# caomw/ClusteringSegmentation-1

Hardware: AMD Instinct MI355X
Metric: Mpixels/sec DivQuant K=256 on 3840x2160 RGB (higher is better)
Workload: dtype u8 RGB (packed u32 frames, planar u8 working buffers), u32/u64 integer sums, f64 updates; 1 GPU; C4 per-GPU share: 8 x 3840x2160 frames per rank per step, K=256, quant_recurse max_iters=10 (cluster + dedup + map), one batched call; engine_lanes=4, gpu_max_hw_queues=8, gpu_max_hw_queues_set_by_bench=True, width=3840, height=2160, k=256, max_iters=10, parallelism=frames-per-rank x1

## Files before the change

### clusteringsegmentation-1_amd/csrc/dq_abi.cpp

```cpp
#include <hip/hip_runtime.h>

#include <algorithm>
#include <cmath>
#include <cstdio>
#include <cstdlib>
#include <cstring>
#include <atomic>
#include <condition_variable>
#include <functional>
#include <mutex>
#include <thread>
#include <unordered_map>
#include <vector>

#include "../../include/DivQuantHeader.h"
#include "../../include/dq_hip.h"
#include "../../include/quant_util.h"
#include "dq_engine.h"
#include "dq_adjacency.h"
#include "dq_merge.h"
#include "dq_regions.h"
#include "dq_weighted.h"

#include <rccl/rccl.h>
// ... 323 lines not shown
  return 0;
}

static int quant_batch(int device, std::vector<dq::FrameJob>& jobs, int max_iters, void* stream) {
  const int nframes = (int)jobs.size();
  const int lanes = std::min(nframes, dq::batch_lanes());
  Engine& e0 = engine_for(device);
  if (lanes <= 1) {
    std::lock_guard<std::mutex> g(e0.mutex());
    e0.run(jobs.data(), nframes, max_iters, true, dev_stream(e0, stream));
  } else {
    DQ_HIP(hipSetDevice(device));
    hipEvent_t ready = events().get();
    DQ_HIP(hipEventRecord(ready, (hipStream_t)stream));
    for (int l = 1; l < lanes; ++l) {
      Engine& e = engine_for(device, l);
      e.set_fixed_point(e0.fixed_point());
      e.set_plan(e0.plan());
      e.set_timing(e0.timing());
    }
    const std::function<void(int)> work = [&](int l) {
      const int f0 = nframes * l / lanes, f1 = nframes * (l + 1) / lanes;
      Engine& e = engine_for(device, l);
      DQ_HIP(hipSetDevice(device));
      std::lock_guard<std::mutex> g(e.mutex());
      DQ_HIP(hipStreamWaitEvent(e.stream(), ready, 0));
      e.run(jobs.data() + f0, f1 - f0, max_iters, true, e.stream());
    };
    lane_workers().run(lanes, work);
    events().put(ready);
    Engine& el = engine_for(device, lanes - 1);
    std::lock_guard<std::mutex> g(e0.mutex());
    uint64_t swept = 0, full = 0, fixes = 0;
    int rounds = 0;
    for (int l = 0; l < lanes; ++l) {
      Engine& e = engine_for(device, l);
      swept += e.last_points_swept;
      full += e.last_points_full;
      fixes += e.last_cursor_fixes;
      rounds = std::max(rounds, e.last_rounds);
      if (l > 0) e0.absorb_stats(e);
    }
    e0.last_means = el.last_means;
    e0.last_sizes = el.last_sizes;
    e0.last_trace = el.last_trace;
    e0.last_rounds = rounds;
    e0.last_points_swept = swept;
    e0.last_points_full = full;
    e0.last_cursor_fixes = fixes;
  }
  int empty = 0;
  for (int i = 0; i < nframes; ++i) empty += jobs[i].num_empty;
  return empty;
}

int dq_hip_quant_batch_dev(int device, int nframes, const uint32_t* const* d_in,
                           const uint32_t* n, uint32_t* const* d_out, uint32_t k,
                           uint32_t* ct, uint32_t* k_out, int max_iters, void* stream) {
  if (nframes <= 0 || !d_in || !n || !d_out || !ct || !k_out || k == 0 || max_iters < 1)
    return -1;
  for (int i = 0; i < nframes; ++i)
    if (!d_in[i] || !d_out[i] || n[i] == 0) return -1;
  std::vector<dq::FrameJob> jobs(nframes);
  for (int i = 0; i < nframes; ++i) {
    jobs[i].d_in = d_in[i];
    jobs[i].n = n[i];
    jobs[i].d_out = d_out[i];
    jobs[i].k = (int)k;
    jobs[i].ct = ct + (size_t)i * k;
  }
  const int empty = quant_batch(device, jobs, max_iters, stream);
  for (int i = 0; i < nframes; ++i) k_out[i] = (uint32_t)jobs[i].k_out;
  return empty;
}

int dq_hip_quant_bgr24_batch_dev(int device, int nframes, const uint8_t* const* d_bgr, uint32_t width,
                                 uint32_t height, uint32_t stride, uint32_t* const* d_out, uint32_t k,
                                 uint32_t* ct, uint32_t* k_out, int uniq, int max_iters, void* stream) {
  if (nframes <= 0 || !d_bgr || !d_out || !ct || !k_out || k == 0 || max_iters < 1 ||
// ... 993 lines not shown
```

### clusteringsegmentation-1_amd/csrc/dq_engine.cpp

```cpp
#include "dq_engine.h"
#include "dq_rules.h"
#include "dq_weighted.h"

#include <rccl/rccl.h>

#include <algorithm>
#include <cfloat>
#include <cmath>
#include <cstdio>
#include <cstdlib>
#include <cstring>
#include <map>
#include <atomic>
#include <chrono>
#include <deque>
#include <functional>
#include <string>
#include <unordered_map>

namespace dq {

void die(const char* what, const char* file, int line, const char* detail) {
  std::fprintf(stderr, "divquant-hip: fatal: %s (%s:%d): %s\n", what, file, line,
               detail ? detail : "");
// ... 395 lines not shown
const uint8_t* Engine::buf_ptr(int buf, const FrameState& f, int shard) const {
  if (buf == BUF_IN) return reinterpret_cast<const uint8_t*>(f.in[shard]);
  return reinterpret_cast<const uint8_t*>(buf == BUF_P0 ? d_p0_ : d_p1_) + f.base[shard];
}

uint64_t Engine::round_tile_len(uint64_t total) const {
  uint64_t tl = (total + tiles_target_ - 1) / tiles_target_;
  tl = ((tl + kSweep - 1) / kSweep) * kSweep;
  return std::max<uint64_t>(kSweep, std::min<uint64_t>(tl, tile_max_));
}

int Engine::src_fmt(const std::vector<int>& ids) const {
  int f = -1;
  for (int id : ids) {
    const Node& n = nodes_[id];
    const int g = n.buf != BUF_IN ? FMT_PLANAR : (frames_[n.frame].job->bgr ? FMT_BGR : FMT_PACKED);
    if (f >= 0 && g != f) return FMT_ANY;
    f = g;
  }
  return f < 0 ? FMT_ANY : f;
}

Engine::RoundBlock Engine::round_block(size_t nr, size_t tiles, size_t ptiles, size_t extra, int max_iters) {
  auto al = [](size_t x) { return (x + 63) & ~(size_t)63; };
  RoundBlock b;
  b.o_tiles = al(nr * sizeof(DevNode));
  b.o_pt = b.o_tiles + al(tiles * sizeof(Tile));
  b.o_extra = b.o_pt + al(ptiles * sizeof(PartTile));
  b.o_ctr = b.o_extra + al(extra);
  b.o_wp = b.o_ctr + al((size_t)(max_iters + 1) * sizeof(LaunchCtr));
  b.o_rd = b.o_wp + al(tiles * kTileWaves * sizeof(uint32_t));
  b.o_sum = b.o_rd + al((size_t)max_iters * nr * sizeof(uint32_t));
  b.o_sd = b.o_sum + al(nr * sizeof(RecSummary));
  b.bytes = b.o_sd + al(nr * sizeof(uint32_t));
  return b;
}

void Engine::round_args(Round& R, char* dblk, const RoundBlock& b, int mode) {
  RoundArgs& ra = R.ra;
  ra.tiles = R.dt;
  ra.nodes = R.dn;
  ra.parts = d_parts_;
  ra.parts2 = d_parts2_;
  ra.wparts = reinterpret_cast<uint32_t*>(dblk + b.o_wp);
  ra.ptiles = reinterpret_cast<const PartTile*>(dblk + b.o_pt);
  ra.sparts = d_sparts_;
  ra.hres = d_res_ + (size_t)R.par * cap_res_;
  ra.ctr = reinterpret_cast<LaunchCtr*>(dblk + b.o_ctr);
  ra.hstat = d_stat_ + (size_t)R.par * cap_stat_;
  ra.seq = R.seq;
  ra.fixed_point = fixed_point_ ? 1 : 0;
  ra.nn = R.nr;
  ra.tot = d_tot_;
  ra.nshard = nshard_;
  ra.debug = debug_;
  ra.rdone = reinterpret_cast<uint32_t*>(dblk + b.o_rd);
  ra.rsum = reinterpret_cast<RecSummary*>(dblk + b.o_sum);
  ra.dres = d_dres_ + (size_t)R.par * cap_res_;
  ra.plane = cap_px_;
  ra.tot_mode = mode;
}

int Engine::enqueue_host_round(const std::vector<int>& active_in, bool root_round, int max_iters,
                               hipStream_t stream) {
  debug_host_delay();
  const double tb0 = trace_ ? host_us() : 0.0;
  const int S = nshard_;
  const int mode = tot_mode();
  rounds_.emplace_back();
  const int ri = (int)rounds_.size() - 1;
  Round& R = rounds_[ri];
  R.root = root_round;
  std::vector<int>& order = R.order;
  std::vector<int>& parents = R.parents;
  slot_of_.assign(nodes_.size(), -1);
  parent_pos_.assign(nodes_.size(), -1);
  for (int id : active_in)
    if (root_round || nodes_[nodes_[id].parent].partitioned) order.push_back(id);
  const int n_own = (int)order.size();
  for (int id : active_in) {
    if (root_round || nodes_[nodes_[id].parent].partitioned) continue;
    order.push_back(id);
    const int p = nodes_[id].parent;
    if (parent_pos_[p] < 0) {
      parent_pos_[p] = (int)parents.size();
      parents.push_back(p);
    }
  }
  const int nl = (int)order.size();
// ... 21 lines not shown
  double own_bytes = 0.0, part_bytes = 0.0;
  for (int a = 0; a < nl; ++a)
    for (int sh = 0; sh < S; ++sh) {
      total += seg(order[a], sh).len;
      if (a < n_own) {
        own_total += seg(order[a], sh).len;
        own_bytes += point_bytes(order[a]) * seg(order[a], sh).len;
      }
    }
  for (int p : parents)
    for (int sh = 0; sh < S; ++sh) {
      parent_total += seg(p, sh).len;
      part_bytes += (point_bytes(p) + 3.0) * seg(p, sh).len;
    }
  const uint64_t tl = round_tile_len(total);
  size_t ntiles = 0, nt_own = 0;
  for (int a = 0; a < nl; ++a) {
    for (int sh = 0; sh < S; ++sh) ntiles += ntiles_of(seg(order[a], sh).len, (uint32_t)tl, (uint32_t)node_tiles_);
    if (a == n_own - 1) nt_own = ntiles;
  }
  size_t nptiles = 0;
  for (int p : parents)
    for (int sh = 0; sh < S; ++sh) nptiles += seg(p, sh).ntiles;
  DQ_CHECK(ntiles <= cap_parts_ && 2 * nptiles <= cap_sparts_, "round larger than the run's tile capacity");
  R.total = total;
  R.own_total = own_total;
  R.parent_total = parent_total;
  R.tl = tl;
  R.ntiles = R.tiles_cap = ntiles;
  R.nptiles = R.ptiles_cap = nptiles;
  R.nt_own = nt_own;

  const RoundBlock blk = round_block((size_t)nr, ntiles, nptiles, nmat * sizeof(PartTile), max_iters);
  const size_t bytes = blk.bytes;
  R.bytes = bytes;
  if (mode == TOT_ALLREDUCE) ensure_totals(nl, stream);
  if (stage_pending_) {
    DQ_HIP(hipEventSynchronize(stage_ev_));
    stage_pending_ = false;
  }
  if (bytes > cap_stage_tab_) {
    DQ_HIP(hipHostFree(h_stage_));
    const size_t c = std::max<size_t>(bytes, 2 * cap_stage_tab_);
    DQ_HIP(hipHostMalloc((void**)&h_stage_, c, hipHostMallocCoherent | hipHostMallocMapped));
    DQ_HIP(hipHostGetDevicePointer((void**)&d_stage_view_, h_stage_, 0));
    cap_stage_tab_ = c;
  }
  char* dblk = arena_alloc(bytes, stream);
  std::memset(h_stage_, 0, bytes);
  DevNode* hn = reinterpret_cast<DevNode*>(h_stage_);
  Tile* ht = reinterpret_cast<Tile*>(h_stage_ + blk.o_tiles);
  PartTile* hp = reinterpret_cast<PartTile*>(h_stage_ + blk.o_pt);
  R.dn = reinterpret_cast<DevNode*>(dblk);
  R.dt = reinterpret_cast<Tile*>(dblk + blk.o_tiles);
  R.tbeg.assign(nr, 0);
  R.tend.assign(nr, 0);

  std::vector<int> pt_first(parents.size() * S);
  {
    int q = 0;
    for (size_t i = 0; i < parents.size(); ++i)
      for (int sh = 0; sh < S; ++sh) {
        pt_first[i * S + sh] = q;
        q += seg(parents[i], sh).ntiles;
      }
  }
  int t = 0;
  for (int a = 0; a < nl; ++a) {
    Node& n = nodes_[order[a]];
    n.queued = true;
    slot_of_[order[a]] = a;
    frames_[n.frame].splits_queued++;
    const FrameState& fs = frames_[n.frame];
    int32_t thr = 0, shift = 0;
    if (!root_round) {
      set_cut(n);
      thr = n.thr;
      shift = 16 - 8 * n.axis;
    }
    for (int sh = 0; sh < S; ++sh) {
      DevNode& d = hn[a * S + sh];
// ... 1756 lines not shown
```

### clusteringsegmentation-1_amd/csrc/dq_engine.h

```cpp
#pragma once
#include <hip/hip_runtime.h>
#include <stdint.h>

#include <condition_variable>
#include <mutex>
#include <queue>
#include <deque>
#include <vector>

#include "dq_internal.h"
#include "dq_kernels.h"
#include "dq_weighted.h"

namespace dq {

[[noreturn]] void die(const char* what, const char* file, int line, const char* detail);
#define DQ_HIP(expr)                                                      \
  do {                                                                    \
    hipError_t e_ = (expr);                                               \
    if (e_ != hipSuccess) ::dq::die(#expr, __FILE__, __LINE__, hipGetErrorString(e_)); \
  } while (0)
#define DQ_CHECK(cond, msg)                                               \
  do {                                                                    \
    if (!(cond)) ::dq::die(#cond, __FILE__, __LINE__, msg);               \
// ... 186 lines not shown
    std::vector<HeapEnt> heap;
    int new_index = 1, old_index = 0;
    int need = -1;
    int splits_queued = 0;
    std::vector<int64_t> trace;
  };

  struct Round {
    uint64_t seq = 0;
    int par = 0;
    bool root = false, planned = false;
    int prev = -1;
    std::vector<int32_t> plist;
    std::vector<int> order;
    std::vector<int> parents;
    int n_own = 0, nl = 0, nr = 0;
    size_t ntiles = 0, nptiles = 0, nt_own = 0;
    size_t tiles_cap = 0, ptiles_cap = 0;
    uint64_t tl = 0;
    uint64_t total = 0, own_total = 0, parent_total = 0;
    std::vector<int32_t> tbeg, tend;
    size_t bytes = 0;
    DevNode* dn = nullptr;
    Tile* dt = nullptr;
    uint32_t* dcounts = nullptr;
    RoundArgs ra{};
    bool kmeans = false;
    bool stats_only = false;
    std::vector<std::pair<size_t, int>> km_events;
    long loop_event = -1;
    double t_enq = 0;
  };
  struct RoundBlock {
    size_t o_tiles, o_pt, o_extra, o_ctr, o_wp, o_rd, o_sum, o_sd, bytes;
  };
  static RoundBlock round_block(size_t nr, size_t tiles, size_t ptiles, size_t extra, int max_iters);
  void round_args(Round& R, char* dblk, const RoundBlock& b, int mode);
  std::deque<Round> rounds_;
  int wait_round_ = -1;

  void ensure_pixels(size_t total);
  void ensure_round(size_t nnodes, size_t ntiles, size_t nptiles, size_t staging_bytes,
                    int max_iters, hipStream_t stream);
  char* arena_alloc(size_t bytes, hipStream_t stream);
  uint32_t wait_status(const uint64_t* slot, uint64_t seq, hipStream_t stream);
  int enqueue_host_round(const std::vector<int>& active, bool root_round, int max_iters,
                         hipStream_t stream);
  bool plan_list(int ri, std::vector<int32_t>* plist);
  int enqueue_planned_round(int prev, const std::vector<int32_t>& plist, int max_iters,
                            hipStream_t stream, const uint32_t* cancel = nullptr);
  void assign_planned(int ri);
  int finish_round(int ri, int max_iters, hipStream_t stream, bool speculate = false, int successor = -1);
  void kmeans_iter(Round& R, int it, int max_iters, hipStream_t stream);
  bool loop_ok(const Round& R) const;
  bool persist_ok(const Round& R) const;
  bool persist_ok_layout(const Round& R) const;
  size_t max_record_tiles(const Round& R) const;
  void kmeans_loop(Round& R, int max_iters, hipStream_t stream, int kind);
  void apply_tune(const char* spec);
  int src_fmt(const std::vector<int>& ids) const;
  void check_arena_zero(hipStream_t stream);
  uint64_t round_tile_len(uint64_t total) const;
  void replay(FrameState& f);
  void next_active(FrameState& f, std::vector<int>* active);
  void finish_frame(FrameState& f, bool last);
  const uint8_t* buf_ptr(int buf, const FrameState& f, int shard) const;
  double point_bytes(int node) const {
// ... 146 lines not shown
```

### clusteringsegmentation-1_amd/csrc/dq_kernels.h

```cpp
#pragma once
#include <hip/hip_runtime.h>
#include <stdint.h>

#include "dq_internal.h"

namespace dq {

constexpr int kBlock = 64 * kTileWaves;
constexpr int kVecPerThread = 4;
constexpr int kSweep = kBlock * kVecPerThread * 4;
constexpr int kWaveSweep = 64 * kVecPerThread * 4;
constexpr uint32_t kMaxTilePx = 16 * kSweep;

constexpr int kCellBits = 5;
constexpr int kCells = 1 << (3 * kCellBits);
constexpr int kCellInline = 7;
constexpr int kCellRecWords = 4;
constexpr int kCellCap = 32;
constexpr uint32_t kCellBrute = 0xFFFF;

enum SrcFmt : int { FMT_PLANAR = 0, FMT_BGR = 1, FMT_PACKED = 2, FMT_ANY = 3 };

struct alignas(16) RecSummary {
  uint32_t off, len, n_new_local, ntiles;
  int32_t tile_begin;
  uint32_t final;
  uint32_t pad[2];
};

struct RoundArgs {
  Tile* tiles;
  DevNode* nodes;
  TilePartial* parts;
  TilePartial* parts2;
  uint32_t* wparts;
  const PartTile* ptiles;
  TilePartial* sparts;
  NodeResult* hres;
  LaunchCtr* ctr;
  uint64_t* hstat;
  uint64_t seq;
  int32_t fixed_point;
  int32_t it;
  int32_t nn;
  uint64_t* tot;
  int32_t nshard;
  int32_t debug;
  uint32_t* rdone;
  NodeResult* dres;
  const uint32_t* counts;
  uint64_t plane;
  int32_t tot_mode;
  int32_t ps_mode;
  RecSummary* rsum;
  uint32_t* sdone;
};

enum PsMode : int32_t { PS_FULL = 0, PS_STATS = 1, PS_LATE = 2, PS_WRITE = 3 };

enum TotMode : int32_t { TOT_OWN = 0, TOT_NODE = 1, TOT_ALLREDUCE = 2 };

struct PlanArgs {
  const DevNode* pn;
  const RecSummary* psum;
  const NodeResult* pres;
  const Tile* ptiles;
  const int32_t* plist;
  int32_t np;
  int32_t node_tiles;
  uint32_t tl;
  uint32_t tiles_cap, ptiles_cap;
  DevNode* cn;
  Tile* ct;
  PartTile* cpt;
  uint32_t* counts;
  uint32_t* hcounts;
  const uint32_t* cancel;
  const uint8_t* p0;
  const uint8_t* p1;
  uint64_t cap_bytes;
  int32_t debug;
  int32_t nshard;
};
constexpr int kPlanMaxParents = 6144;

constexpr int32_t kDebugPrewarm = 1, kDebugUneven = 2, kDebugHostDelay = 4, kDebugPlanStall = 8,
                  kDebugArenaCheck = 16, kDebugFreshArena = 32;
void launch_plan(const PlanArgs& a, hipStream_t stream);
void launch_plansplit(const PlanArgs& pa, const RoundArgs& a, int grid, int fmt, hipStream_t stream);
void launch_upload(void* dst, const void* src_dev_view, size_t bytes, hipStream_t stream);
void launch_zero(void* dst, size_t bytes, hipStream_t stream);
struct SumSrcs { const uint64_t* p[kMaxShard]; };
void launch_sum_u64(const SumSrcs& src, int nsrc, uint64_t* dst, size_t count, hipStream_t stream);

void launch_pass(int kind, const RoundArgs& a, int ntiles, hipStream_t stream);
void launch_kpass(int kind, const RoundArgs& a, int ntiles, hipStream_t stream);
void launch_epilogue(int kind, const RoundArgs& a, int nnodes, hipStream_t stream);
void launch_fix_cursors(const RoundArgs& a, int ntiles, hipStream_t stream);
void launch_nodesum(int kind, const RoundArgs& a, int nlogical, hipStream_t stream);
constexpr uint32_t kLoopMaxTiles = 1024;
constexpr uint32_t kLoopMaxLen = 61440u * 16u - 32u;
void launch_kloop(const RoundArgs& a, int nrec, int max_iters, hipStream_t stream);
void launch_kpersist(const RoundArgs& a, int ntiles, int max_iters, hipStream_t stream);
void launch_partsplit(const RoundArgs& a, int nptiles, int fmt, hipStream_t stream);

struct alignas(16) MapTask {
  const uint32_t* in;
  uint32_t* out;
  const uint32_t* pal;
  const uint16_t* lut;
  uint32_t* cell_rec;
  uint16_t* cell_idx;
  uint32_t* cell_c32;
  uint32_t n;
  int32_t k;
  uint32_t block_begin;
  uint32_t grp_per_block;
  int32_t bgr;
  int32_t labels;
};
static_assert(sizeof(MapTask) == 80, "the label width fills MapTask's padding: the colour kernels' task loads are unchanged");
constexpr uint32_t map_label_off(uint32_t k) { return (k + 3u) & ~3u; }

void launch_build_cells(const MapTask* tasks, int ntasks, int kmax, hipStream_t stream);
uint32_t map_groups_per_block(uint32_t n);
void launch_map(const MapTask* tasks, int ntasks, int kmax, uint32_t nblocks, hipStream_t stream,
                int labels = 0);
constexpr int kMapLdsBlock = 1024;
void launch_map_lds(const MapTask* tasks, int ntasks, int kmax, uint32_t nblocks, bool bgr,
                    hipStream_t stream, int labels = 0);

struct BlockHistArgs {
  const uint32_t* quant;
  uint32_t width, height, block_w, block_h;
  uint32_t* mode;
  uint32_t* ndistinct;
// ... 19 lines not shown
```

### clusteringsegmentation-1_amd/csrc/dq_kernels.hip

```cpp
#include <hip/hip_runtime.h>

#include <type_traits>

#include "dq_kernels.h"
#include "dq_rules.h"
#include "stl_order.h"

namespace dq {

namespace {

typedef uint32_t u32x4 __attribute__((ext_vector_type(4)));
typedef const __attribute__((address_space(1))) uint32_t g_cu32;
typedef const __attribute__((address_space(1))) u32x4 g_cu4;
typedef __attribute__((address_space(1))) uint32_t g_u32;
__device__ __forceinline__ g_cu4* as_g4(const uint32_t* p) { return (g_cu4*)p; }
__device__ __forceinline__ g_cu32* as_g(const uint32_t* p) { return (g_cu32*)p; }
__device__ __forceinline__ g_u32* as_gw(uint32_t* p) { return (g_u32*)p; }

__device__ __forceinline__ uint32_t lane_id() { return threadIdx.x & 63; }
__device__ __forceinline__ uint32_t wave_id() { return __builtin_amdgcn_readfirstlane(threadIdx.x >> 6); }

__device__ __forceinline__ uint32_t mbcnt64(uint64_t m) {
  return __builtin_amdgcn_mbcnt_hi((uint32_t)(m >> 32),
// ... 223 lines not shown
    add_sums(w, vm & cut_new_mask(w, (uint32_t)q.shift, q.thr), s);
  } else {
    add_sums(w, vm & ~old_mask(w, vm, q, exact_all), s);
  }
}

template <int KIND, bool PLANAR, bool BGR = false>
__device__ __forceinline__ void wave_pass(const uint8_t* src, uint64_t plane, uint32_t ws, uint32_t we,
                                          const Params& q, LaneSums& s) {
  const bool exact_all = !(q.eps < __builtin_inff());
  uint32_t vs = ws & ~15u;
  bool full = vs >= ws && vs + kWaveSweep <= we;
  RawSweep x;
  if (vs < we) {
    if (full) fetch_sweep<PLANAR, true, false, BGR>(src, plane, vs, we, x);
    else fetch_sweep<PLANAR, false, false, BGR>(src, plane, vs, we, x);
  }
  while (vs < we) {
    Sweep w;
    unpack_sweep<PLANAR, BGR>(x, w);
    const uint32_t nvs = vs + kWaveSweep;
    const bool nfull = nvs + kWaveSweep <= we;
    if (nvs < we) {
      if (nfull) fetch_sweep<PLANAR, true, false, BGR>(src, plane, nvs, we, x);
      else fetch_sweep<PLANAR, false, false, BGR>(src, plane, nvs, we, x);
    }
    if (full) sweep_sums<KIND, PLANAR, true>(w, vs, ws, we, q, exact_all, s);
    else sweep_sums<KIND, PLANAR, false>(w, vs, ws, we, q, exact_all, s);
    vs = nvs;
    full = nfull;
  }
}

__device__ void node_results(NodeResult* r, const DevNode* w, const uint64_t t[F_NUM],
                             const double om[3], const double nm[3], double nw, double ow) {
  const double s = w->s, tw = w->tw;
  double nv[3], ov[3];
  for (int c = 0; c < 3; ++c) {
    double q = (double)t[F_QR + c];
    q *= s;
    nv[c] = q / nw - nm[c] * nm[c];
  }
  for (int c = 0; c < 3; ++c) {
    const double dn = nm[c] - w->tm[c];
    const double dox = om[c] - w->tm[c];
    ov[c] = ((tw * w->tv[c] - nw * (nv[c] + dn * dn)) / ow) - dox * dox;
  }
  for (int c = 0; c < 3; ++c) {
    r->om[c] = om[c];
    r->nm[c] = nm[c];
    r->nv[c] = nv[c];
    r->ov[c] = ov[c];
  }
  r->nw = nw;
  r->ow = ow;
  r->tse_old = ow * (ov[0] + ov[1] + ov[2]);
  r->tse_new = nw * (nv[0] + nv[1] + nv[2]);
  r->n_new = t[F_CNT];
}

template <int KIND>
__device__ bool node_update(DevNode* w, NodeResult* r, const uint64_t t[F_NUM], bool fixed_point) {
  const double s = w->s, tw = w->tw;
  if (KIND == PASS_INIT) {
    double tm[3], tv[3];
    for (int c = 0; c < 3; ++c) {
// ... 136 lines not shown
#pragma unroll
  for (int k = 0; k < F_NUM; ++k) acc[k] = wave_sum_u64(acc[k]);
  if (lane_id() == 0) {
#pragma unroll
    for (int k = 0; k < F_NUM; ++k) red[wave_id()][k] = acc[k];
  }
  __syncthreads();
  if (threadIdx.x == 0) {
    for (int k = 0; k < F_NUM; ++k) {
      tot[k] = 0;
      for (int v = 0; v < kBlock / 64; ++v) tot[k] += red[v][k];
    }
  }
}

template <int KIND>
__global__ __launch_bounds__(kBlock) void nodesum_kernel(RoundArgs a) {
  constexpr bool kMeans = KIND == PASS_KMEANS || KIND == PASS_KLAST;
  if (a.counts && a.counts[2] != 0) return;
  __shared__ uint64_t red[kBlock / 64][8];
  const DevNode* w0 = a.nodes + (size_t)blockIdx.x * a.nshard;
  uint64_t acc[7] = {0, 0, 0, 0, 0, 0, 0};
  if (!(kMeans && w0->done_it != 0))
    for (int sh = 0; sh < a.nshard; ++sh) sum_record<KIND>(a, w0 + sh, acc);
  uint64_t tot[7];
  block_sum7(acc, red, tot);
  if (threadIdx.x == 0) {
    uint64_t* g = a.tot + (size_t)blockIdx.x * 8;
    for (int k = 0; k < F_NUM; ++k) g[k] = tot[k];
    g[7] = 0;
  }
}

template <bool COHERENT = false>
__device__ __forceinline__ void record_cursors(Tile* tiles, const uint32_t* wp, int tb, int te,
                                               uint32_t lane) {
  const int T = te - tb;
  const int chunk = (T + 63) / 64;
  const int c0 = tb + (int)lane * chunk;
  const int c1 = min(te, c0 + chunk);
  auto ld = [&](int i) -> uint32_t {
    if (COHERENT) return __hip_atomic_load(wp + i, __ATOMIC_RELAXED, __HIP_MEMORY_SCOPE_AGENT);
    return wp[i];
  };
  uint64_t local = 0;
  for (int i = c0; i < c1; ++i)
    for (int ww = 0; ww < kTileWaves; ++ww) {
      const uint32_t x = ld(i * kTileWaves + ww);
      local += (uint64_t)(x & 0xFFFFu) | ((uint64_t)(x >> 16) << 32);
    }
  uint64_t inc = local;
#pragma unroll
  for (int o = 1; o < 64; o <<= 1) {
    const uint64_t u = __shfl_up(inc, o, 64);
    if (lane >= (uint32_t)o) inc += u;
  }
  const uint64_t run0 = inc - local;
  uint32_t ro = (uint32_t)run0, rn = (uint32_t)(run0 >> 32);
  for (int i = c0; i < c1; ++i)
    for (int ww = 0; ww < kTileWaves; ++ww) {
      const uint32_t x = ld(i * kTileWaves + ww);
      tiles[i].old_base[ww] = ro;
      tiles[i].new_base[ww] = rn;
      ro += x & 0xFFFFu;
      rn += x >> 16;
    }
}

template <int W>
__device__ __forceinline__ void block_cursors(Tile* tiles, const uint32_t* wp, int tb, int te,
                                              uint64_t* s_tot, int wbase = 0) {
  const int T = te - tb;
  const int chunk = (T + W - 1) / W;
  const int c0 = tb + (int)threadIdx.x * chunk;
  const int c1 = min(te, c0 + chunk);
  const uint32_t lane = lane_id(), wv = wave_id();
  uint64_t local = 0;
  for (int i = c0; i < c1; ++i) {
    const u32x4 x = *(const u32x4*)(wp + (size_t)(i - wbase) * kTileWaves);
#pragma unroll
    for (int ww = 0; ww < kTileWaves; ++ww) local += (uint64_t)(x[ww] & 0xFFFFu) | ((uint64_t)(x[ww] >> 16) << 32);
  }
  uint64_t inc = local;
#pragma unroll
  for (int o = 1; o < 64; o <<= 1) {
    const uint64_t u = __shfl_up(inc, o, 64);
    if (lane >= (uint32_t)o) inc += u;
  }
  if (lane == 63) s_tot[wv] = inc;
  __syncthreads();
  uint64_t base = 0;
  for (uint32_t w = 0; w < wv; ++w) base += s_tot[w];
  const uint64_t run0 = base + inc - local;
  uint32_t ro = (uint32_t)run0, rn = (uint32_t)(run0 >> 32);
  for (int i = c0; i < c1; ++i) {
    const u32x4 x = *(const u32x4*)(wp + (size_t)(i - wbase) * kTileWaves);
    u32x4 ob, nb;
#pragma unroll
    for (int ww = 0; ww < kTileWaves; ++ww) {
// ... 117 lines not shown
      fin = node_update<KIND>(w, &sres, tot, a.fixed_point != 0) ? 1 : 0;
      if (fin) {
        for (int c = 0; c < 3; ++c) { sres.tm[c] = w->tm[c]; sres.tv[c] = w->tv[c]; }
        w->n_new_local = local_new;
        sres.n_new_local = local_new;
        sres.done_it = w->done_it;
      }
    }
    s_fin = fin;
  }
  __syncthreads();
  if (!skip && threadIdx.x < (uint32_t)kW16)
    ((g_u4*)gw)[threadIdx.x] = reinterpret_cast<const u32x4*>(&sw)[threadIdx.x];
  const bool final_results = s_fin != 0;
  if ((kMeans || KIND == PASS_SPLIT) && final_results) {
    if (stage_wp) block_cursors<kEpiBlock>(a.tiles, s_wp, tb, te, s_tot, tb);
    else block_cursors<kEpiBlock>(a.tiles, a.wparts, tb, te, s_tot);
  }
  if (wave_id() != 0) return;
  if (kMeans || KIND == PASS_SPLIT) {
    if ((a.debug & kDebugUneven) && debug_unlucky(blockIdx.x)) debug_sleep_us(10);
    __builtin_amdgcn_fence(__ATOMIC_RELEASE, "wavefront");
    __builtin_amdgcn_wave_barrier();
    __builtin_amdgcn_fence(__ATOMIC_ACQUIRE, "wavefront");
    if (final_results)
      store_result(a.hres + blockIdx.x, a.dres ? a.dres + blockIdx.x : nullptr, sres, lane, w->len, a.seq,
                   a.rsum ? a.rsum + blockIdx.x : nullptr, w);
    asm volatile("s_waitcnt vmcnt(0)" ::: "memory");
    if (lane == 0)
      arrive(a.ctr + a.it, blockIdx.x, (uint32_t)a.nn, !skip && !final_results, a.hstat + a.it, a.seq);
  }
}

template <int KIND>
__device__ __forceinline__ void kmeans_epilogue_wave(const RoundArgs& a, int node, NodeResult* sres, int it_arr,
                                                     bool final_only) {
  const int S = a.nshard, r0 = node * S;
  const uint32_t lane = lane_id();
  const uint32_t* pp = reinterpret_cast<const uint32_t*>(a.parts);
  uint64_t tot[F_NUM] = {0, 0, 0, 0, 0, 0, 0};
  uint32_t my_new = 0;
  for (int sh = 0; sh < S; ++sh) {
    const DevNode* w = a.nodes + r0 + sh;
    const int tb = w->tile_begin, te = w->tile_end;
    uint64_t acc[F_NUM] = {0, 0, 0, 0, 0, 0, 0};
    for (int i = tb + (int)lane; i < te; i += 64)
#pragma unroll
      for (int k = 0; k < F_NUM; ++k)
        acc[k] += __hip_atomic_load(pp + (size_t)i * 8 + k, __ATOMIC_RELAXED, __HIP_MEMORY_SCOPE_AGENT);
#pragma unroll
    for (int k = 0; k < F_NUM; ++k) {
      const uint64_t v = wave_sum_u64(acc[k]);
      tot[k] += v;
      if (k == F_CNT && lane == (uint32_t)sh) my_new = (uint32_t)v;
    }
  }
  if (a.tot_mode == TOT_ALLREDUCE) {
    if (lane < (uint32_t)F_NUM + 1) {
      uint64_t v = 0;
#pragma unroll
      for (int k = 0; k < F_NUM; ++k) v = lane == (uint32_t)k ? tot[k] : v;
      a.tot[(size_t)node * 8 + lane] = v;
    }
    return;
  }
  int fin = 0;
  if (lane < (uint32_t)S) {
    DevNode* w = a.nodes + r0 + lane;
    NodeResult* r = sres + lane;
    fin = node_update<KIND>(w, r, tot, a.fixed_point != 0) ? 1 : 0;
    if (fin) {
      for (int c = 0; c < 3; ++c) { r->tm[c] = w->tm[c]; r->tv[c] = w->tv[c]; }
      w->n_new_local = my_new;
      r->n_new_local = my_new;
      r->done_it = w->done_it;
    }
  }
  const bool final_results = __shfl(fin, 0, 64) != 0;
  __builtin_amdgcn_fence(__ATOMIC_RELEASE, "wavefront");
  __builtin_amdgcn_wave_barrier();
  __builtin_amdgcn_fence(__ATOMIC_ACQUIRE, "wavefront");
  if (final_results) {
// ... 48 lines not shown
  }
  if ((a.debug & kDebugUneven) && debug_unlucky(blockIdx.x)) debug_sleep_us(10);
  if (lane_id() == 0) {
    __hip_atomic_store(a.wparts + blockIdx.x * kTileWaves + wave_id(),
                       (vsum - f[F_CNT]) | (f[F_CNT] << 16), __ATOMIC_RELAXED, __HIP_MEMORY_SCOPE_AGENT);
#pragma unroll
    for (int k = 0; k < 8; ++k) red[wave_id()][k] = k < F_NUM ? f[k] : 0u;
  }
  __syncthreads();
  if (threadIdx.x < 8) {
    uint32_t x = 0;
#pragma unroll
    for (int w = 0; w < kBlock / 64; ++w) x += red[w][threadIdx.x];
    __hip_atomic_store(a.parts[blockIdx.x].f + threadIdx.x, x, __ATOMIC_RELAXED, __HIP_MEMORY_SCOPE_AGENT);
  }
  asm volatile("s_waitcnt vmcnt(0)" ::: "memory");
  __syncthreads();
  if (threadIdx.x == 0) {
    const int ntiles = S == 1 ? nd.tile_end - nd.tile_begin
                              : a.nodes[node * S + S - 1].tile_end - a.nodes[node * S].tile_begin;
    const bool last = __hip_atomic_fetch_add(a.rdone + (size_t)a.it * a.nn + node, 1u, __ATOMIC_RELEASE,
                                             __HIP_MEMORY_SCOPE_AGENT) == (uint32_t)ntiles - 1;
    if (last) {
      __builtin_amdgcn_fence(__ATOMIC_ACQUIRE, "agent");
      asm volatile("s_waitcnt vmcnt(0)" ::: "memory");
    }
    slast = last;
  }
  __syncthreads();
  if (slast && wave_id() == 0) kmeans_epilogue_wave<KIND>(a, node, sres, a.it, false);
}

constexpr uint32_t kPersistSpin = 1u << 26;

__device__ __forceinline__ Params uniform_params(const Params& p) {
  Params q;
  const uint32_t* s = reinterpret_cast<const uint32_t*>(&p);
  uint32_t* d = reinterpret_cast<uint32_t*>(&q);
#pragma unroll
  for (int i = 0; i < (int)(sizeof(Params) / 4); ++i) d[i] = (uint32_t)__builtin_amdgcn_readfirstlane(s[i]);
  return q;
}

__global__ __launch_bounds__(kBlock, kPassWaves) void kpersist_kernel(RoundArgs a, int32_t max_iters) {
  typedef __attribute__((address_space(1))) u32x4 g_u4;
  const Tile t = a.tiles[blockIdx.x];
  const int rec = t.node;
  DevNode* gw = a.nodes + rec;
  const uint32_t lane = lane_id();
  __shared__ __attribute__((aligned(16))) DevNode sw;
  __shared__ NodeResult sres;
  __shared__ uint32_t red[kBlock / 64][8];
  __shared__ int sgo, sfin;
  static_assert(sizeof(DevNode) % 16 == 0, "the record is staged in 16-B words");
  constexpr int kW16 = (int)(sizeof(DevNode) / 16);
  if (threadIdx.x < (uint32_t)kW16) reinterpret_cast<u32x4*>(&sw)[threadIdx.x] = ((const g_cu4*)gw)[threadIdx.x];
  __syncthreads();
  const int tb = sw.tile_begin, te = sw.tile_end;
  const int ntiles = te - tb;
  const bool lead = (int)blockIdx.x == tb;
  if (sw.done_it != 0) {
    if (lead && threadIdx.x == 0)
      arrive(a.ctr + (max_iters - 1), (uint32_t)rec, (uint32_t)a.nn, false, a.hstat + (max_iters - 1), a.seq);
    return;
  }
  const uintptr_t srcw = (uintptr_t)sw.src;
  const uint8_t* src = (const uint8_t*)(((uintptr_t)(uint32_t)__builtin_amdgcn_readfirstlane((uint32_t)(srcw >> 32)) << 32) |
                                        (uint32_t)__builtin_amdgcn_readfirstlane((uint32_t)srcw));
  for (int it = 0; it < max_iters; ++it) {
    const bool klast = it == max_iters - 1;
    TilePartial* parts = (it & 1) ? a.parts2 : a.parts;
    const Params q = uniform_params(sw.prm);
    LaneSums s;
    uint32_t ws, we;
    wave_range(t.start, t.end, wave_id(), ws, we);
    wave_pass<PASS_KMEANS, true>(src, a.plane, ws, we, q, s);
    uint32_t f[8] = {s.cnt, s.sr, s.sg, s.sb, s.qr, s.qg, s.qb, 0};
#pragma unroll
    for (int k = 0; k < F_NUM; ++k) f[k] = wave_sum_u32(f[k]);
    const uint32_t vsum = wave_sum_u32(s.vcnt);
    if (lane == 0) {
      __hip_atomic_store(a.wparts + blockIdx.x * kTileWaves + wave_id(),
                         (vsum - f[F_CNT]) | (f[F_CNT] << 16), __ATOMIC_RELAXED, __HIP_MEMORY_SCOPE_AGENT);
#pragma unroll
      for (int k = 0; k < 8; ++k) red[wave_id()][k] = k < F_NUM ? f[k] : 0u;
    }
    __syncthreads();
    if (threadIdx.x < 8) {
      uint32_t x = 0;
#pragma unroll
      for (int w = 0; w < kBlock / 64; ++w) x += red[w][threadIdx.x];
      __hip_atomic_store(parts[blockIdx.x].f + threadIdx.x, x, __ATOMIC_RELAXED, __HIP_MEMORY_SCOPE_AGENT);
    }
    if ((a.debug & kDebugUneven) && debug_unlucky(blockIdx.x + 131u * (uint32_t)it)) debug_sleep_us(10);
    if ((a.debug & kDebugPrewarm) && wave_id() == 0) {
      const uint32_t* pp = reinterpret_cast<const uint32_t*>(parts);
      uint32_t x = 0;
      for (int i = tb + (int)lane; i < te; i += 64)
        for (int k = 0; k < 8; ++k) x += pp[(size_t)i * 8 + k];
      asm volatile("s_waitcnt vmcnt(0)" ::"v"(x) : "memory");
    }
    asm volatile("s_waitcnt vmcnt(0)" ::: "memory");
    __syncthreads();
    uint32_t* word = a.rdone + (size_t)it * a.nn + rec;
    if (threadIdx.x == 0) {
      int go = 1;
      if (__hip_atomic_fetch_add(word, 1u, __ATOMIC_RELEASE, __HIP_MEMORY_SCOPE_AGENT) != (uint32_t)ntiles - 1u) {
        for (uint32_t spin = 0;
             __hip_atomic_load(word, __ATOMIC_RELAXED, __HIP_MEMORY_SCOPE_AGENT) != (uint32_t)ntiles; ++spin) {
          if (spin == kPersistSpin) {
            go = 0;
            break;
          }
          __builtin_amdgcn_s_sleep(2);
        }
      }
      __builtin_amdgcn_fence(__ATOMIC_ACQUIRE, "agent");
      asm volatile("s_waitcnt vmcnt(0)" ::: "memory");
      sgo = go;
    }
    __syncthreads();
    if (!sgo) return;
    if (wave_id() == 0) {
      const uint32_t* pp = reinterpret_cast<const uint32_t*>(parts);
      uint64_t tot[F_NUM] = {0, 0, 0, 0, 0, 0, 0};
      for (int i = tb + (int)lane; i < te; i += 64)
#pragma unroll
        for (int k = 0; k < F_NUM; ++k)
          tot[k] += __hip_atomic_load(pp + (size_t)i * 8 + k, __ATOMIC_RELAXED, __HIP_MEMORY_SCOPE_AGENT);
#pragma unroll
      for (int k = 0; k < F_NUM; ++k) tot[k] = wave_sum_u64(tot[k]);
      if (lane == 0) {
        const bool fin = klast ? node_update<PASS_KLAST>(&sw, &sres, tot, a.fixed_point != 0)
                               : node_update<PASS_KMEANS>(&sw, &sres, tot, a.fixed_point != 0);
        if (fin) {
          for (int c = 0; c < 3; ++c) { sres.tm[c] = sw.tm[c]; sres.tv[c] = sw.tv[c]; }
          sw.n_new_local = (uint32_t)tot[F_CNT];
          sres.n_new_local = (uint32_t)tot[F_CNT];
          sres.done_it = sw.done_it;
        }
        sfin = fin ? 1 : 0;
      }
    }
    __syncthreads();
    if (sfin) {
      if (lead && wave_id() == 0) {
        if (lane < (uint32_t)kW16) ((g_u4*)gw)[lane] = reinterpret_cast<const u32x4*>(&sw)[lane];
        record_cursors<true>(a.tiles, a.wparts, tb, te, lane);
        store_result(a.hres + rec, a.dres ? a.dres + rec : nullptr, sres, lane, sw.len, a.seq,
                     a.rsum ? a.rsum + rec : nullptr, &sw);
        asm volatile("s_waitcnt vmcnt(0)" ::: "memory");
        if (lane == 0)
          arrive(a.ctr + (max_iters - 1), (uint32_t)rec, (uint32_t)a.nn, false, a.hstat + (max_iters - 1), a.seq);
      }
      return;
    }
  }
}

struct ChunkAcc {
  bool on;
  uint32_t off, len, tl;
  uint32_t* w0;
  uint32_t k, t0, tend, q;
  uint32_t w, end;
  uint32_t acc;
  uint32_t lnew;
};

__device__ __forceinline__ void chunk_tile(ChunkAcc& c) {
  c.t0 = c.off + c.k * c.tl;
  c.tend = min(c.t0 + c.tl, c.off + c.len);
  c.q = ((c.tend - c.t0 + kSweep - 1) / kSweep) * kWaveSweep;
}

struct ChildInfo {
  uint32_t off, len, tl, tb;
  int32_t on;
};

__device__ __forceinline__ ChildInfo child_info(const DevNode* nodes, int rec) {
// ... 2201 lines not shown
```

Before: 61600 Mpix/s.

## Replace persistent-kernel counter barrier with tagged granule exchange and prefetched sweeps

For records spanning at most 32 tiles, the persistent k-means kernel now publishes each tile's partial sums and per-wave counts as tagged 64-bit granules in a per-round buffer, instead of using a shared arrival counter. Every tile polls its peers' granules until all tags match, with no separate atomic barrier or acquire fence. The planar sweep is also software-pipelined: the first sweep is fetched before the iteration loop and the next sweep is fetched while the current one is summed. Non-granule partial reads switch to vectorized loads. This trades extra device memory and tag-polling traffic for fewer serialized atomic round trips per iteration. Stats aggregation also gains a persist-rounds counter.

```diff
diff --git a/clusteringsegmentation-1_amd/csrc/dq_abi.cpp b/clusteringsegmentation-1_amd/csrc/dq_abi.cpp
--- a/clusteringsegmentation-1_amd/csrc/dq_abi.cpp
+++ b/clusteringsegmentation-1_amd/csrc/dq_abi.cpp
@@ -379,9 +379,10 @@
     Engine& el = engine_for(device, lanes - 1);
     std::lock_guard<std::mutex> g(e0.mutex());
     uint64_t swept = 0, full = 0, fixes = 0;
-    int rounds = 0;
+    int rounds = 0, persist = 0;
     for (int l = 0; l < lanes; ++l) {
       Engine& e = engine_for(device, l);
+      persist += e.last_persist_rounds;
       swept += e.last_points_swept;
       full += e.last_points_full;
       fixes += e.last_cursor_fixes;
@@ -392,6 +393,7 @@
     e0.last_sizes = el.last_sizes;
     e0.last_trace = el.last_trace;
     e0.last_rounds = rounds;
+    e0.last_persist_rounds = persist;
     e0.last_points_swept = swept;
     e0.last_points_full = full;
     e0.last_cursor_fixes = fixes;
diff --git a/clusteringsegmentation-1_amd/csrc/dq_engine.cpp b/clusteringsegmentation-1_amd/csrc/dq_engine.cpp
--- a/clusteringsegmentation-1_amd/csrc/dq_engine.cpp
+++ b/clusteringsegmentation-1_amd/csrc/dq_engine.cpp
@@ -451,7 +451,9 @@
   b.o_rd = b.o_wp + al(tiles * kTileWaves * sizeof(uint32_t));
   b.o_sum = b.o_rd + al((size_t)max_iters * nr * sizeof(uint32_t));
   b.o_sd = b.o_sum + al(nr * sizeof(RecSummary));
-  b.bytes = b.o_sd + al(nr * sizeof(uint32_t));
+  b.o_gr = (b.o_sd + al(nr * sizeof(uint32_t)) + 127) & ~(size_t)127;
+  const bool gran = tiles <= (size_t)kPersistGranuleTiles * nr;
+  b.bytes = b.o_gr + (gran ? tiles * kPersistGranuleTileBytes : 0);
   return b;
 }
 
@@ -474,6 +476,7 @@
   ra.nshard = nshard_;
   ra.debug = debug_;
   ra.rdone = reinterpret_cast<uint32_t*>(dblk + b.o_rd);
+  ra.gran = b.bytes > b.o_gr ? reinterpret_cast<uint64_t*>(dblk + b.o_gr) : nullptr;
   ra.rsum = reinterpret_cast<RecSummary*>(dblk + b.o_sum);
   ra.dres = d_dres_ + (size_t)R.par * cap_res_;
   ra.plane = cap_px_;
@@ -561,8 +564,8 @@
   R.nt_own = nt_own;
 
   const RoundBlock blk = round_block((size_t)nr, ntiles, nptiles, nmat * sizeof(PartTile), max_iters);
-  const size_t bytes = blk.bytes;
-  R.bytes = bytes;
+  const size_t bytes = blk.o_gr;
+  R.bytes = blk.bytes;
   if (mode == TOT_ALLREDUCE) ensure_totals(nl, stream);
   if (stage_pending_) {
     DQ_HIP(hipEventSynchronize(stage_ev_));
@@ -575,7 +578,7 @@
     DQ_HIP(hipHostGetDevicePointer((void**)&d_stage_view_, h_stage_, 0));
     cap_stage_tab_ = c;
   }
-  char* dblk = arena_alloc(bytes, stream);
+  char* dblk = arena_alloc(blk.bytes, stream);
   std::memset(h_stage_, 0, bytes);
   DevNode* hn = reinterpret_cast<DevNode*>(h_stage_);
   Tile* ht = reinterpret_cast<Tile*>(h_stage_ + blk.o_tiles);
diff --git a/clusteringsegmentation-1_amd/csrc/dq_engine.h b/clusteringsegmentation-1_amd/csrc/dq_engine.h
--- a/clusteringsegmentation-1_amd/csrc/dq_engine.h
+++ b/clusteringsegmentation-1_amd/csrc/dq_engine.h
@@ -242,7 +242,7 @@
     double t_enq = 0;
   };
   struct RoundBlock {
-    size_t o_tiles, o_pt, o_extra, o_ctr, o_wp, o_rd, o_sum, o_sd, bytes;
+    size_t o_tiles, o_pt, o_extra, o_ctr, o_wp, o_rd, o_sum, o_sd, o_gr, bytes;
   };
   static RoundBlock round_block(size_t nr, size_t tiles, size_t ptiles, size_t extra, int max_iters);
   void round_args(Round& R, char* dblk, const RoundBlock& b, int mode);
diff --git a/clusteringsegmentation-1_amd/csrc/dq_kernels.h b/clusteringsegmentation-1_amd/csrc/dq_kernels.h
--- a/clusteringsegmentation-1_amd/csrc/dq_kernels.h
+++ b/clusteringsegmentation-1_amd/csrc/dq_kernels.h
@@ -47,6 +47,7 @@
   int32_t nshard;
   int32_t debug;
   uint32_t* rdone;
+  uint64_t* gran;
   NodeResult* dres;
   const uint32_t* counts;
   uint64_t plane;
@@ -102,6 +103,9 @@
 constexpr uint32_t kLoopMaxLen = 61440u * 16u - 32u;
 void launch_kloop(const RoundArgs& a, int nrec, int max_iters, hipStream_t stream);
 void launch_kpersist(const RoundArgs& a, int ntiles, int max_iters, hipStream_t stream);
+constexpr int kPersistGranuleTiles = 32;
+constexpr int kPersistGranuleLine = 16;
+constexpr size_t kPersistGranuleTileBytes = 2 * kPersistGranuleLine * 8;
 void launch_partsplit(const RoundArgs& a, int nptiles, int fmt, hipStream_t stream);
 
 struct alignas(16) MapTask {
diff --git a/clusteringsegmentation-1_amd/csrc/dq_kernels.hip b/clusteringsegmentation-1_amd/csrc/dq_kernels.hip
--- a/clusteringsegmentation-1_amd/csrc/dq_kernels.hip
+++ b/clusteringsegmentation-1_amd/csrc/dq_kernels.hip
@@ -279,6 +279,45 @@
   }
 }
 
+__device__ __forceinline__ void planar_first_sweep(const uint8_t* src, uint64_t plane, uint32_t ws, uint32_t we,
+                                                   u32x4 (&h)[3]) {
+  const uint32_t vs = ws & ~15u;
+  RawSweep x;
+#pragma unroll
+  for (int c = 0; c < 3; ++c) x.v[c] = (u32x4){0u, 0u, 0u, 0u};
+  if (vs < we) {
+    if (vs >= ws && vs + kWaveSweep <= we) fetch_sweep<true, true>(src, plane, vs, we, x);
+    else fetch_sweep<true, false>(src, plane, vs, we, x);
+  }
+#pragma unroll
+  for (int c = 0; c < 3; ++c) h[c] = x.v[c];
+}
+
+template <int KIND>
+__device__ __forceinline__ void planar_pass_from(const uint8_t* src, uint64_t plane, uint32_t ws, uint32_t we,
+                                                 const Params& q, const u32x4 (&h)[3], LaneSums& s) {
+  const bool exact_all = !(q.eps < __builtin_inff());
+  uint32_t vs = ws & ~15u;
+  bool full = vs >= ws && vs + kWaveSweep <= we;
+  RawSweep x;
+#pragma unroll
+  for (int c = 0; c < 3; ++c) x.v[c] = h[c];
+  while (vs < we) {
+    Sweep w;
+    unpack_sweep<true>(x, w);
+    const uint32_t nvs = vs + kWaveSweep;
+    const bool nfull = nvs + kWaveSweep <= we;
+    if (nvs < we) {
+      if (nfull) fetch_sweep<true, true>(src, plane, nvs, we, x);
+      else fetch_sweep<true, false>(src, plane, nvs, we, x);
+    }
+    if (full) sweep_sums<KIND, true, true>(w, vs, ws, we, q, exact_all, s);
+    else sweep_sums<KIND, true, false>(w, vs, ws, we, q, exact_all, s);
+    vs = nvs;
+    full = nfull;
+  }
+}
+
 __device__ void node_results(NodeResult* r, const DevNode* w, const uint64_t t[F_NUM],
                              const double om[3], const double nm[3], double nw, double ow) {
   const double s = w->s, tw = w->tw;
@@ -481,21 +520,16 @@
   }
 }
 
-template <bool COHERENT = false>
-__device__ __forceinline__ void record_cursors(Tile* tiles, const uint32_t* wp, int tb, int te,
-                                               uint32_t lane) {
+template <typename LD>
+__device__ __forceinline__ void record_cursors_from(Tile* tiles, int tb, int te, uint32_t lane, LD ld) {
   const int T = te - tb;
   const int chunk = (T + 63) / 64;
   const int c0 = tb + (int)lane * chunk;
   const int c1 = min(te, c0 + chunk);
-  auto ld = [&](int i) -> uint32_t {
-    if (COHERENT) return __hip_atomic_load(wp + i, __ATOMIC_RELAXED, __HIP_MEMORY_SCOPE_AGENT);
-    return wp[i];
-  };
   uint64_t local = 0;
   for (int i = c0; i < c1; ++i)
     for (int ww = 0; ww < kTileWaves; ++ww) {
-      const uint32_t x = ld(i * kTileWaves + ww);
+      const uint32_t x = ld(i, ww);
       local += (uint64_t)(x & 0xFFFFu) | ((uint64_t)(x >> 16) << 32);
     }
   uint64_t inc = local;
@@ -508,12 +542,21 @@
   uint32_t ro = (uint32_t)run0, rn = (uint32_t)(run0 >> 32);
   for (int i = c0; i < c1; ++i)
     for (int ww = 0; ww < kTileWaves; ++ww) {
-      const uint32_t x = ld(i * kTileWaves + ww);
+      const uint32_t x = ld(i, ww);
       tiles[i].old_base[ww] = ro;
       tiles[i].new_base[ww] = rn;
       ro += x & 0xFFFFu;
       rn += x >> 16;
     }
+}
+
+template <bool COHERENT = false>
+__device__ __forceinline__ void record_cursors(Tile* tiles, const uint32_t* wp, int tb, int te,
+                                               uint32_t lane) {
+  record_cursors_from(tiles, tb, te, lane, [&](int i, int ww) -> uint32_t {
+    if (COHERENT) return __hip_atomic_load(wp + i * kTileWaves + ww, __ATOMIC_RELAXED, __HIP_MEMORY_SCOPE_AGENT);
+    return wp[i * kTileWaves + ww];
+  });
 }
 
 template <int W>
@@ -697,6 +740,18 @@
   }
 }
 
+__device__ __forceinline__ void add_partial(const uint32_t* pp, int i, uint64_t acc[F_NUM]) {
+  const g_cu4* p4 = (const g_cu4*)pp + 2 * (size_t)i;
+  const u32x4 x = p4[0], y = p4[1];
+  acc[0] += x[0];
+  acc[1] += x[1];
+  acc[2] += x[2];
+  acc[3] += x[3];
+  acc[4] += y[0];
+  acc[5] += y[1];
+  acc[6] += y[2];
+}
+
 template <int KIND>
 __device__ __forceinline__ void kmeans_epilogue_wave(const RoundArgs& a, int node, NodeResult* sres, int it_arr,
                                                      bool final_only) {
@@ -709,10 +764,7 @@
     const DevNode* w = a.nodes + r0 + sh;
     const int tb = w->tile_begin, te = w->tile_end;
     uint64_t acc[F_NUM] = {0, 0, 0, 0, 0, 0, 0};
-    for (int i = tb + (int)lane; i < te; i += 64)
-#pragma unroll
-      for (int k = 0; k < F_NUM; ++k)
-        acc[k] += __hip_atomic_load(pp + (size_t)i * 8 + k, __ATOMIC_RELAXED, __HIP_MEMORY_SCOPE_AGENT);
+    for (int i = tb + (int)lane; i < te; i += 64) add_partial(pp, i, acc);
 #pragma unroll
     for (int k = 0; k < F_NUM; ++k) {
       const uint64_t v = wave_sum_u64(acc[k]);
@@ -827,6 +879,52 @@
 }
 
 constexpr uint32_t kPersistSpin = 1u << 26;
+
+typedef __attribute__((address_space(1))) uint64_t g_u64;
+__device__ __forceinline__ uint32_t granule_at(int tile, int par, int g) {
+  return ((uint32_t)tile * 2u + (uint32_t)par) * (uint32_t)kPersistGranuleLine + (uint32_t)g;
+}
+
+template <int PER, int N>
+__device__ __forceinline__ bool sweep_granules(uint64_t* gran, int tb, int ntiles, int par, int first,
+                                               uint32_t tag, uint32_t lane, uint32_t (&v)[N]) {
+  static_assert(N * 64 >= kPersistGranuleTiles * PER, "a pass covers the largest record");
+  const int ng = ntiles * PER;
+  const g_u64* base = (const g_u64*)gran;
+  uint32_t p[N];
+#pragma unroll
+  for (int k = 0; k < N; ++k) {
+    const int g = min((int)lane + 64 * k, ng - 1);
+    p[k] = granule_at(tb + g / PER, par, first + g % PER);
+  }
+  for (uint32_t spin = 0;; ++spin) {
+    uint64_t x[N];
+#pragma unroll
+    for (int k = 0; k < N; ++k) x[k] = __hip_atomic_load(base + p[k], __ATOMIC_RELAXED, __HIP_MEMORY_SCOPE_AGENT);
+    bool ok = true;
+#pragma unroll
+    for (int k = 0; k < N; ++k) {
+      v[k] = (uint32_t)x[k];
+      ok = ok && (uint32_t)(x[k] >> 32) == tag;
+    }
+    if (__all(ok)) return true;
+    if (spin == kPersistSpin) return false;
+    __builtin_amdgcn_s_sleep(1);
+  }
+}
+
+__device__ __forceinline__ int persist_update(DevNode* sw, NodeResult* sres, const uint64_t tot[F_NUM], bool klast,
+                                              bool fixed_point) {
+  const bool fin = klast ? node_update<PASS_KLAST>(sw, sres, tot, fixed_point)
+                         : node_update<PASS_KMEANS>(sw, sres, tot, fixed_point);
+  if (fin) {
+    for (int c = 0; c < 3; ++c) { sres->tm[c] = sw->tm[c]; sres->tv[c] = sw->tv[c]; }
+    sw->n_new_local = (uint32_t)tot[F_CNT];
+    sres->n_new_local = (uint32_t)tot[F_CNT];
+    sres->done_it = sw->done_it;
+  }
+  return fin ? 1 : 0;
+}
 
 __device__ __forceinline__ Params uniform_params(const Params& p) {
   Params q;
@@ -862,86 +960,139 @@
   const uintptr_t srcw = (uintptr_t)sw.src;
   const uint8_t* src = (const uint8_t*)(((uintptr_t)(uint32_t)__builtin_amdgcn_readfirstlane((uint32_t)(srcw >> 32)) << 32) |
                                         (uint32_t)__builtin_amdgcn_readfirstlane((uint32_t)srcw));
+  const bool use_gran = a.gran != nullptr && ntiles <= kPersistGranuleTiles;
+  uint32_t ws, we;
+  wave_range(t.start, t.end, wave_id(), ws, we);
+  u32x4 hx[3];
+  planar_first_sweep(src, a.plane, ws, we, hx);
   for (int it = 0; it < max_iters; ++it) {
     const bool klast = it == max_iters - 1;
-    TilePartial* parts = (it & 1) ? a.parts2 : a.parts;
+    const int par = it & 1;
+    const uint32_t tag = (uint32_t)it + 1u;
+    TilePartial* parts = par ? a.parts2 : a.parts;
     const Params q = uniform_params(sw.prm);
     LaneSums s;
-    uint32_t ws, we;
-    wave_range(t.start, t.end, wave_id(), ws, we);
-    wave_pass<PASS_KMEANS, true>(src, a.plane, ws, we, q, s);
+    planar_pass_from<PASS_KMEANS>(src, a.plane, ws, we, q, hx, s);
     uint32_t f[8] = {s.cnt, s.sr, s.sg, s.sb, s.qr, s.qg, s.qb, 0};
 #pragma unroll
     for (int k = 0; k < F_NUM; ++k) f[k] = wave_sum_u32(f[k]);
     const uint32_t vsum = wave_sum_u32(s.vcnt);
     if (lane == 0) {
-      __hip_atomic_store(a.wparts + blockIdx.x * kTileWaves + wave_id(),
-                         (vsum - f[F_CNT]) | (f[F_CNT] << 16), __ATOMIC_RELAXED, __HIP_MEMORY_SCOPE_AGENT);
-#pragma unroll
-      for (int k = 0; k < 8; ++k) red[wave_id()][k] = k < F_NUM ? f[k] : 0u;
+      const uint32_t cw = (vsum - f[F_CNT]) | (f[F_CNT] << 16);
+      if (!use_gran)
+        __hip_atomic_store(a.wparts + blockIdx.x * kTileWaves + wave_id(), cw, __ATOMIC_RELAXED, __HIP_MEMORY_SCOPE_AGENT);
+#pragma unroll
+      for (int k = 0; k < 8; ++k) red[wave_id()][k] = k < F_NUM ? f[k] : cw;
     }
     __syncthreads();
-    if (threadIdx.x < 8) {
-      uint32_t x = 0;
-#pragma unroll
-      for (int w = 0; w < kBlock / 64; ++w) x += red[w][threadIdx.x];
-      __hip_atomic_store(parts[blockIdx.x].f + threadIdx.x, x, __ATOMIC_RELAXED, __HIP_MEMORY_SCOPE_AGENT);
-    }
-    if ((a.debug & kDebugUneven) && debug_unlucky(blockIdx.x + 131u * (uint32_t)it)) debug_sleep_us(10);
-    if ((a.debug & kDebugPrewarm) && wave_id() == 0) {
-      const uint32_t* pp = reinterpret_cast<const uint32_t*>(parts);
-      uint32_t x = 0;
-      for (int i = tb + (int)lane; i < te; i += 64)
-        for (int k = 0; k < 8; ++k) x += pp[(size_t)i * 8 + k];
-      asm volatile("s_waitcnt vmcnt(0)" ::"v"(x) : "memory");
-    }
-    asm volatile("s_waitcnt vmcnt(0)" ::: "memory");
+    if (use_gran) {
+      if (wave_id() == 0) {
+        if (a.debug & kDebugPrewarm) {
+          uint64_t x = 0;
+          for (int i = tb; i < te; ++i)
+            x += ((const g_u64*)a.gran)[granule_at(i, par, (int)(lane & 15u))];
+          asm volatile("s_waitcnt vmcnt(0)" ::"v"(x) : "memory");
+        }
+        if ((a.debug & kDebugUneven) && debug_unlucky(blockIdx.x + 131u * (uint32_t)it)) debug_sleep_us(10);
+        if (lane < 12u) {
+          uint32_t x = 0;
+          if (lane < (uint32_t)F_NUM) {
+#pragma unroll
+            for (int w = 0; w < kBlock / 64; ++w) x += red[w][lane];
+          } else if (lane >= 8u) {
+            x = red[lane - 8u][7];
+          }
+          __hip_atomic_store((g_u64*)a.gran + granule_at((int)blockIdx.x, par, (int)lane), ((uint64_t)tag << 32) | x,
+                             __ATOMIC_RELAXED, __HIP_MEMORY_SCOPE_AGENT);
+        }
+        constexpr int kN = kPersistGranuleTiles * 8 / 64;
+        uint32_t v[kN];
+        const bool go = sweep_granules<8>(a.gran, tb, ntiles, par, 0, tag, lane, v);
+        uint64_t acc = 0;
+#pragma unroll
+        for (int k = 0; k < kN; ++k)
+          if ((int)lane + 64 * k < ntiles * 8) acc += v[k];
+#pragma unroll
+        for (int o = 8; o < 64; o <<= 1) acc += __shfl_xor(acc, o, 64);
+        uint64_t tot[F_NUM];
+#pragma unroll
+        for (int k = 0; k < F_NUM; ++k) tot[k] = __shfl(acc, k, 64);
+        if (lane == 0) sfin = go ? persist_update(&sw, &sres, tot, klast, a.fixed_point != 0) : 2;
+      }
+    } else {
+      if (threadIdx.x < 8) {
+        uint32_t x = 0;
+#pragma unroll
+        for (int w = 0; w < kBlock / 64; ++w) x += red[w][threadIdx.x];
+        if (threadIdx.x == 7) x = 0;
+        __hip_atomic_store(parts[blockIdx.x].f + threadIdx.x, x, __ATOMIC_RELAXED, __HIP_MEMORY_SCOPE_AGENT);
+      }
+      if ((a.debug & kDebugUneven) && debug_unlucky(blockIdx.x + 131u * (uint32_t)it)) debug_sleep_us(10);
+      if ((a.debug & kDebugPrewarm) && wave_id() == 0) {
+        const uint32_t* pp = reinterpret_cast<const uint32_t*>(parts);
+        uint32_t x = 0;
+        for (int i = tb + (int)lane; i < te; i += 64)
+          for (int k = 0; k < 8; ++k) x += pp[(size_t)i * 8 + k];
+        asm volatile("s_waitcnt vmcnt(0)" ::"v"(x) : "memory");
+      }
+      asm volatile("s_waitcnt vmcnt(0)" ::: "memory");
+      __syncthreads();
+      uint32_t* word = a.rdone + (size_t)it * a.nn + rec;
+      if (threadIdx.x == 0) {
+        int go = 1;
+        if (__hip_atomic_fetch_add(word, 1u, __ATOMIC_RELEASE, __HIP_MEMORY_SCOPE_AGENT) != (uint32_t)ntiles - 1u) {
+          for (uint32_t spin = 0;
+               __hip_atomic_load(word, __ATOMIC_RELAXED, __HIP_MEMORY_SCOPE_AGENT) != (uint32_t)ntiles; ++spin) {
+            if (spin == kPersistSpin) {
+              go = 0;
+              break;
+            }
+            __builtin_amdgcn_s_sleep(2);
+          }
+        }
+        __builtin_amdgcn_fence(__ATOMIC_ACQUIRE, "agent");
+        asm volatile("s_waitcnt vmcnt(0)" ::: "memory");
+        sgo = go;
+      }
+      __syncthreads();
+      if (!sgo) return;
+      if (wave_id() == 0) {
+        const uint32_t* pp = reinterpret_cast<const uint32_t*>(parts);
+        uint64_t tot[F_NUM] = {0, 0, 0, 0, 0, 0, 0};
+        for (int i = tb + (int)lane; i < te; i += 64) add_partial(pp, i, tot);
+#pragma unroll
+        for (int k = 0; k < F_NUM; ++k) tot[k] = wave_sum_u64(tot[k]);
+        if (lane == 0) sfin = persist_update(&sw, &sres, tot, klast, a.fixed_point != 0);
+      }
+    }
     __syncthreads();
-    uint32_t* word = a.rdone + (size_t)it * a.nn + rec;
-    if (threadIdx.x == 0) {
-      int go = 1;
-      if (__hip_atomic_fetch_add(word, 1u, __ATOMIC_RELEASE, __HIP_MEMORY_SCOPE_AGENT) != (uint32_t)ntiles - 1u) {
-        for (uint32_t spin = 0;
-             __hip_atomic_load(word, __ATOMIC_RELAXED, __HIP_MEMORY_SCOPE_AGENT) != (uint32_t)ntiles; ++spin) {
-          if (spin == kPersistSpin) {
-            go = 0;
-            break;
-          }
-          __builtin_amdgcn_s_sleep(2);
-        }
-      }
-      __builtin_amdgcn_fence(__ATOMIC_ACQUIRE, "agent");
-      asm volatile("s_waitcnt vmcnt(0)" ::: "memory");
-      sgo = go;
-    }
-    __syncthreads();
-    if (!sgo) return;
-    if (wave_id() == 0) {
-      const uint32_t* pp = reinterpret_cast<const uint32_t*>(parts);
-      uint64_t tot[F_NUM] = {0, 0, 0, 0, 0, 0, 0};
-      for (int i = tb + (int)lane; i < te; i += 64)
-#pragma unroll
-        for (int k = 0; k < F_NUM; ++k)
-          tot[k] += __hip_atomic_load(pp + (size_t)i * 8 + k, __ATOMIC_RELAXED, __HIP_MEMORY_SCOPE_AGENT);
-#pragma unroll
-      for (int k = 0; k < F_NUM; ++k) tot[k] = wave_sum_u64(tot[k]);
-      if (lane == 0) {
-        const bool fin = klast ? node_update<PASS_KLAST>(&sw, &sres, tot, a.fixed_point != 0)
-                               : node_update<PASS_KMEANS>(&sw, &sres, tot, a.fixed_point != 0);
-        if (fin) {
-          for (int c = 0; c < 3; ++c) { sres.tm[c] = sw.tm[c]; sres.tv[c] = sw.tv[c]; }
-          sw.n_new_local = (uint32_t)tot[F_CNT];
-          sres.n_new_local = (uint32_t)tot[F_CNT];
-          sres.done_it = sw.done_it;
-        }
-        sfin = fin ? 1 : 0;
-      }
-    }
-    __syncthreads();
+    if (sfin == 2) return;
     if (sfin) {
       if (lead && wave_id() == 0) {
         if (lane < (uint32_t)kW16) ((g_u4*)gw)[lane] = reinterpret_cast<const u32x4*>(&sw)[lane];
-        record_cursors<true>(a.tiles, a.wparts, tb, te, lane);
+        if (use_gran) {
+          static_assert(kPersistGranuleTiles <= 64 && kTileWaves == 4, "one tile per lane, four count granules");
+          constexpr int kN = kPersistGranuleTiles * 4 / 64;
+          uint32_t cv[kN];
+          if (!sweep_granules<4>(a.gran, tb, ntiles, par, 8, tag, lane, cv)) return;
+          uint32_t cw[kTileWaves];
+#pragma unroll
+          for (int ww = 0; ww < kTileWaves; ++ww) {
+            const int g = 4 * min((int)lane, ntiles - 1) + ww;
+            uint32_t x = 0;
+#pragma unroll
+            for (int k = 0; k < kN; ++k) {
+              const uint32_t y = __shfl(cv[k], g & 63, 64);
+              if ((g >> 6) == k) x = y;
+            }
+            cw[ww] = x;
+          }
+          record_cursors_from(a.tiles, tb, te, lane, [&](int, int ww) -> uint32_t {
+            return ww == 0 ? cw[0] : ww == 1 ? cw[1] : ww == 2 ? cw[2] : cw[3];
+          });
+        } else {
+          record_cursors<true>(a.tiles, a.wparts, tb, te, lane);
+        }
         store_result(a.hres + rec, a.dres ? a.dres + rec : nullptr, sres, lane, sw.len, a.seq,
                      a.rsum ? a.rsum + rec : nullptr, &sw);
         asm volatile("s_waitcnt vmcnt(0)" ::: "memory");
```

Result: no change. 61880 Mpix/s, median of 4 (+0.5%).
